# vislearn/HINT

Hardware: AMD Instinct MI355X
Metric: train_samples_per_sec (higher is better)
Workload: dtype f32; 1 GPU; power_hint_8: d=6, 8 recursive coupling blocks, c_internal=[140, 70, 35, 17], batch 4096 per GPU; global_batch=4096, parallelism=dp1, hip_graph=True, steps_per_graph=1, input=batch resident in the captured step's input buffer (no per-step copy), rccl_world_size=1, backend=none (one process), gradient_allreduce=none (one process: clamp + Adam ride in the weight gradients' final reduction)

## Files before the change

hint_amd/_lib.py:

```python
from __future__ import annotations

import ctypes as C
import os

_HERE = os.path.dirname(os.path.abspath(__file__))
LIB_PATH = os.environ.get("HINT_AMD_LIB") or os.path.join(_HERE, "lib", "libhint_amd.so")
ABI_VERSION = 8


class HintAmdError(RuntimeError):
    pass


class AdamSeg(C.Structure):
    _fields_ = [("p", C.c_void_p), ("g", C.c_void_p), ("m", C.c_void_p), ("v", C.c_void_p), ("n", C.c_int64)]


class NodeDesc(C.Structure):
    _fields_ = [("off", C.c_int32), ("D", C.c_int32), ("k", C.c_int32), ("r", C.c_int32),
                ("h", C.c_int32), ("depth", C.c_int32), ("p_off", C.c_int64 * 12)]


class MmdDesc(C.Structure):
    _fields_ = [("x", C.c_void_p), ("y", C.c_void_p), ("n_x", C.c_int32), ("n_y", C.c_int32), ("d", C.c_int32),
# ... 60 lines not shown
    "hint_build_info": (C.c_char_p, []),
    "hint_debug_set_prefetch": (C.c_int, [C.c_int]),
    "hint_debug_reload_knobs": (C.c_int, []),
    "hint_debug_last_lds_bytes": (C.c_int32, [C.c_int32]),
    "hint_plan_create": (C.c_int, [C.POINTER(NodeDesc), C.c_int32, C.c_int32, C.c_int32, C.c_float,
                                   C.POINTER(C.c_void_p)]),
    "hint_plan_check": (C.c_int, [C.POINTER(NodeDesc), C.c_int32, C.c_int32, C.c_int32, C.c_float,
                                  C.POINTER(C.c_int64)]),
    "hint_plan_destroy": (None, [C.c_void_p]),
    "hint_plan_param_floats": (C.c_int64, [C.c_void_p]),
    "hint_plan_packed_floats": (C.c_int64, [C.c_void_p]),
    "hint_plan_tape_floats": (C.c_int64, [C.c_void_p, C.c_int32]),
    "hint_plan_workspace_bytes": (C.c_size_t, [C.c_void_p, C.c_int32]),
    "hint_plan_lds_bytes": (C.c_int32, [C.c_void_p, C.c_int32]),
    "hint_plan_describe": (C.c_int, [C.c_void_p, C.c_int32, C.POINTER(C.c_int32)]),
    "hint_plan_dispatch": (C.c_int, [C.c_void_p, C.c_int32, C.POINTER(C.c_int32), C.c_int32]),
    "hint_plan_check_dispatch": (C.c_int, [C.POINTER(NodeDesc), C.c_int32, C.c_int32, C.c_int32, C.c_float, C.c_int32,
                                           C.c_int32, C.POINTER(C.c_int32), C.c_int32]),
    "hint_plan_paths": (C.c_int, [C.c_void_p, C.c_int32, C.POINTER(C.c_int32), C.c_int32]),
    "hint_plan_check_paths": (C.c_int, [C.POINTER(NodeDesc), C.c_int32, C.c_int32, C.c_int32, C.c_float, C.c_int32,
                                        C.c_int32, C.POINTER(C.c_int32), C.c_int32]),
    "hint_plan_check_digest": (C.c_int, [C.POINTER(NodeDesc), C.c_int32, C.c_int32, C.c_int32, C.c_float,
                                         C.POINTER(C.c_uint64), C.c_int32]),
    "hint_block_pack": (C.c_int, [C.c_void_p] * 4),
    "hint_pack_group_create": (C.c_int, [C.POINTER(C.c_void_p), C.POINTER(C.c_void_p), C.POINTER(C.c_void_p),
                                         C.c_int32, C.POINTER(C.c_void_p)]),
    "hint_pack_group_run": (C.c_int, [C.c_void_p, C.c_void_p]),
    "hint_pack_group_run_ex": (C.c_int, [C.c_void_p, C.c_void_p, C.c_int32, C.c_void_p, C.c_void_p, C.c_void_p]),
    "hint_pack_group_destroy": (None, [C.c_void_p]),
    "hint_block_forward": (C.c_int, [C.c_void_p] * 8 + [C.c_int32, C.c_void_p]),
    "hint_block_inverse": (C.c_int, [C.c_void_p] * 7 + [C.c_int32, C.c_void_p]),
    "hint_block_backward": (C.c_int, [C.c_void_p] * 11 + [C.c_int32, C.c_void_p, C.c_size_t, C.c_int32,
                                                          C.c_void_p]),
    "hint_block_forward_ex": (C.c_int, [C.c_void_p] * 11 + [C.c_int32, C.c_void_p]),
    "hint_block_inverse_ex": (C.c_int, [C.c_void_p] * 9 + [C.c_int32, C.c_void_p]),
    "hint_block_backward_ex": (C.c_int, [C.c_void_p] * 11 + [C.c_int32, C.c_void_p, C.c_size_t, C.c_void_p,
                                                             C.c_float, C.c_float, C.c_int32, C.c_void_p]),
    "hint_plan_inverse_workspace_bytes": (C.c_size_t, [C.c_void_p, C.c_int32]),
    "hint_block_inverse_backward": (C.c_int, [C.c_void_p] * 9 + [C.c_int32, C.c_void_p, C.c_size_t, C.c_void_p, C.c_int32,
                                                                 C.c_void_p]),
    "hint_chain_create": (C.c_int, [C.c_void_p, C.c_int32, C.c_int32, C.POINTER(C.c_void_p)]),
    "hint_chain_set_block": (C.c_int, [C.c_void_p, C.c_int32] + [C.c_void_p] * 5 + [C.c_size_t, C.c_void_p]),
    "hint_chain_commit": (C.c_int, [C.c_void_p]),
    "hint_chain_forward": (C.c_int, [C.c_void_p] * 8),
    "hint_chain_forward_noisy": (C.c_int, [C.c_void_p] * 7 + [C.c_float, C.c_void_p, C.c_void_p, C.c_void_p]),
    "hint_chain_backward": (C.c_int, [C.c_void_p] * 7 + [C.c_float, C.c_float, C.c_int32, C.c_void_p]),
# ... 77 lines not shown
```

hint_amd/csrc/hint_abi.cpp:

```cpp
#include "hint_host.hpp"

#include <atomic>

using namespace hint;

static thread_local std::string g_err;
static unsigned long long* g_stamp_buf = nullptr;

namespace hint {

static Knobs read_knobs() {
    Knobs k;
    auto get = [&](const char* name, int* out) {
        const char* e = std::getenv(name);
        if (!e || !*e) return false;
        *out = std::atoi(e);
        k.non_default += (k.non_default.empty() ? "" : " ") + std::string(name) + "=" + e;
        return true;
    };
    int v;
    if (get("HINT_PLAN_DUMP", &v)) k.plan_dump = v != 0;
    if (get("HINT_WL", &v)) k.wl = v != 0;
    if (get("HINT_WL_NR", &v)) k.wl_nr = v;
    if (get("HINT_SUB", &v)) k.sub = v != 0;
    if (get("HINT_NW", &v)) k.nw = v;
    if (get("HINT_LEAN", &v)) k.lean = v != 0;
    if (get("HINT_LEANW", &v)) k.leanw = v != 0;
    if (get("HINT_LEANW_MAX", &v)) k.leanw_max = std::min(std::max(v, 4), LEANW_MAX);
    if (get("HINT_FUSE_DW1", &v)) k.fuse_dw1 = v != 0;
    if (get("HINT_PF", &v)) k.pf = v != 0 ? 1 : 0;
    if (get("HINT_NO_BWD_FLY", &v)) k.no_bwd_fly = v != 0;
    if (get("HINT_DW_SPLITS", &v)) k.dw_splits = v;
    if (get("HINT_DW_SMALL", &v)) k.dw_small = v != 0 ? 1 : 0;
    if (get("HINT_ABLATION_OK", &v)) k.ablation_ok = v != 0;
    return k;
}
static std::mutex g_knobs_mu;
static Knobs* g_knobs = nullptr;
const Knobs& knobs() {
    std::lock_guard<std::mutex> lk(g_knobs_mu);
    if (!g_knobs) g_knobs = new Knobs(read_knobs());
    return *g_knobs;
}

int fail(const char* fmt, ...) {
    char buf[512];
    va_list ap;
    va_start(ap, fmt);
    vsnprintf(buf, sizeof buf, fmt, ap);
    va_end(ap);
    g_err = buf;
    return 1;
}
std::string& last_error_ref() { return g_err; }

const hint_plan* variant(const hint_plan* P, int B) {
// ... 175 lines not shown
    if (!knobs().ablation_ok) return fail("this is an ablation build (HINT_ABLATE_STORE): its gradients are wrong; set HINT_ABLATION_OK=1 for timing runs");
#endif

    const Dispatch D = dispatch(P, B, n_total);
    P = D.P;
    if ((parts & 1) && D.bwd == BWD_WL) {
        KArgs a = make_args(P, B, true);
        const int nr = D.nr;
        WlArgs w = P->wl_b[nr - 1];
        bool any_perm = one.perm != nullptr;
        if (chain_host) for (int i = 0; i < n_chain; ++i) any_perm = any_perm || chain_host[i].perm != nullptr;
        const int lds = lds_with_perms(P, plan_lds(P, true, nr), n_chain, any_perm, &a, true);
        w.off_perm = a.perm_lds;
        HIP_TRY(launch_wl_bwd(a, w, lds, D.grid, one, chain, n_chain, x, g_z, g_J, g_x, gz_scale, gJ_const, s));
    } else if (parts & 1) {
        KArgs a = make_args(P, B, true);
        const int lds = add_sink(P, P->lds_bwd, &a);
        g_last_lds[1].store(lds, std::memory_order_relaxed);
        HIP_TRY((D.bwd == BWD_FLY ? launch_bwd_fly : D.bwd == BWD_N3 ? launch_bwd_n3 : launch_bwd)(a, lds, D.grid, one, chain, n_chain, x, c,
                                                               g_z, g_J, g_x, g_c, gz_scale, gJ_const, s));
    }
    if (!(parts & 2)) return 0;
    const int splits = D.dw_splits, rows_per_wg = D.dw_rows;
    HIP_TRY(launch_wgrad(P->d_wjobs, P->n_wjobs, P->wsorted ? -P->n_wsmall - 1 : P->n_wsmall, splits, one, chain, n_chain, cb0, P->WT, P->ST, P->d, P->dc, P->n_levels, B,
                         rows_padded(B), rows_per_wg, act_stride(P, B), P->lean ? 0 : act_stride(P, B),
                         (P->lean ? 1 : 2) * act_stride(P, B) * 4 + bits_stride(P, B), P->param_floats, x, c, P->d_real,
                         accumulate, P->fuse_dw1 ? P->d_twmap : nullptr, P->tw_floats, ws_thin_off(P, B), D.grid,
                         P->num_cu, adam, D.dw_small, D.dw_wide, s));
    return 0;
}

}

static int apply(const hint_plan* P, bool rev, const float* params, const float* packed, const float* x,
                 const float* c, float* z, float* J, float* tape, const float* perm, const float* J_in,
                 float* loss_acc, int32_t B, void* stream, float noise = 0.f, const uint64_t* rng_state = nullptr,
                 float* x_noisy = nullptr) {
    const char* what = rev ? "inverse" : "forward";
    if (!P || !params || !packed || !x || !z || !J) return fail("hint_block_%s: null argument", what);
    if (P->dc > 0 && !c) return fail("hint_block_%s: plan has dc=%d but c is NULL", what, P->dc);
    if (B < 0) return fail("negative batch");
    if (B == 0) return 0;
    const Dispatch D = dispatch(P, B);
    P = D.P;
    ChainBlock one{};
    one.params = params; one.packed = packed; one.perm = perm;
    bind_tape(P, B, rev ? nullptr : tape, &one);
// ... 407 lines not shown
```

hint_amd/csrc/hint_dev.h:

```cpp
#pragma once
#include <stdint.h>

namespace hint {

constexpr int ROWS = 16;
constexpr int TILE = 16;
#ifndef HINT_MAX_NW
#define HINT_MAX_NW 8
#endif
#ifndef HINT_NTT
#define HINT_NTT 3
#endif
constexpr int MAX_NW = HINT_MAX_NW;
constexpr int NTT = HINT_NTT;
constexpr int MAX_RT = 4;
constexpr int MAX_CT = 12;
constexpr int LEANW_MAX = 28;
constexpr int LV_REGS = 4;

constexpr int PACK_SLACK = 1024;
struct PackSeg {
    int64_t dst;
    int64_t src;
    int32_t N, K;
// ... 47 lines not shown
struct Group {
    int32_t unit_begin, unit_end, ntiles, row_begin;
    int32_t ent_begin, ent_cnt, rng_begin, level;
    int32_t level_last, gcol0, gcols, lop_begin;
    int32_t level_first, tile_begin, wcol0, lean;
};
static_assert(sizeof(Group) == 64, "Group must be 4 x 16 bytes");

struct Ent {
    int16_t xcol, nquad;
    int16_t sl_ns, sl_nt;
    int32_t s_off, t_off;
};
static_assert(sizeof(Ent) == 16, "Ent must be 16 bytes");

struct LaneOp {
    int16_t sc_unit, sc_k;
    int16_t cp_ls, cp_lt;
    int16_t cp_gs, cp_gt;
    int32_t pad;
};
static_assert(sizeof(LaneOp) == 16, "LaneOp must be 16 bytes");

enum { WSRC_G1 = 0, WSRC_G2 = 1, WSRC_GST = 2, WSRC_A1 = 3, WSRC_A2 = 4, WSRC_X = 5, WSRC_C = 6, WSRC_A1R = 7, WSRC_G2R = 8 };
struct WJob {
    int32_t psrc, pcol, M, mw;
    int32_t qsrc, qcol, N, nw;
    int32_t qlevel, ldo;
    int32_t pmax, qmax;
    int64_t wofs;
    int64_t bofs;
    int32_t r_w1, r_b1;
    int32_t r_w3;
    int32_t r_cin, r_xoff;
    int32_t r_r, r_gcol;
    int32_t r_h, r_wcol;
    int32_t pad_[7];
};
static_assert(sizeof(WJob) == 128, "WJob must be 128 bytes");

struct RowRec {
    int32_t base1, base2;
    int32_t counts;
    int32_t aux;
    int32_t ocol;
    int32_t tile;
    int32_t slab;
// ... 95 lines not shown
```

hint_amd/csrc/hint_host.hpp:

```cpp
#pragma once
#include <hip/hip_runtime.h>

#include <algorithm>
#include <cmath>
#include <cstdarg>
#include <cstdio>
#include <cstdlib>
#include <cstring>
#include <mutex>
#include <string>
#include <vector>

#include "../../include/hint_amd.h"
#include "hint_dev.h"
#include "hint_adam.hpp"

namespace hint {
hipError_t launch_pack(const PackSeg* segs, const int2* ptiles, int n_tiles, const int32_t* bmap, int n_bias,
                       long bias_off, const float* params, float* packed, hipStream_t stream);
hipError_t launch_pack_many(const PackItem* items, int n_items, int grid, float* zero_buf, int zero_floats,
                            unsigned long long* rng_state, float* opt_state, hipStream_t stream);
hipError_t launch_zero(float* p, long n, int num_cu, hipStream_t stream);
hipError_t launch_inv_lane(int op, float* out, const float* g, const float* a, const float* b, const uint8_t* lower, long n, int d,
                           int num_cu, hipStream_t stream);
hipError_t launch_inv_minus(float* dst, const float* src, long n, int keep, int num_cu, hipStream_t stream);
hipError_t launch_inv_rowmat(const float* x, const float* P, float* y, long n, int d, int num_cu, hipStream_t stream);
hipError_t launch_apply(bool rev, bool fly, const KArgs& a, int lds_bytes, int grid, const ChainBlock& one,
                        const ChainBlock* chain, int n_chain, const float* x, const float* c, float* z, float* J,
                        const float* J_in, float* loss_acc, float noise, const unsigned long long* rng_state,
                        float* x_noisy, hipStream_t stream);
hipError_t launch_bwd(const KArgs& a, int lds_bytes, int grid, const ChainBlock& one, const ChainBlock* chain,
                      int n_chain, const float* x, const float* c, const float* g_z, const float* g_J,
                      float* g_x, float* g_c, float gz_scale, float gJ_const, hipStream_t stream);
hipError_t launch_wgrad(const WJob* jobs, int n_jobs, int n_small, int splits, const ChainBlock& one, const ChainBlock* chain,
                        int n_chain, int cb0, int WT, int ST, int d, int dc, int n_levels, int B, int Bp, int rows_per_wg,
                        int64_t act_stride, int64_t a2_off, int64_t bits_a2_off, int64_t param_floats, const float* x,
                        const float* c, const uint8_t* real, int accumulate, const int32_t* twmap, int tw_floats,
                        int64_t thin_slab_off, int thin_slabs, int num_cu, const AdamFuse* adam, bool small, bool wide,
                        hipStream_t stream);
hipError_t launch_bwd_n3(const KArgs& a, int lds_bytes, int grid, const ChainBlock& one, const ChainBlock* chain,
                         int n_chain, const float* x, const float* c, const float* g_z, const float* g_J,
                         float* g_x, float* g_c, float gz_scale, float gJ_const, hipStream_t stream);
hipError_t set_max_lds_apply(int bytes);
hipError_t launch_ext_coeff(const ExtArgs& a, hipStream_t stream);
hipError_t set_max_lds_bwd(int bytes);
hipError_t set_max_lds_bwd_n3(int bytes);
hipError_t launch_bwd_fly(const KArgs& a, int lds_bytes, int grid, const ChainBlock& one, const ChainBlock* chain,
                          int n_chain, const float* x, const float* c, const float* g_z, const float* g_J,
                          float* g_x, float* g_c, float gz_scale, float gJ_const, hipStream_t stream);
hipError_t set_max_lds_bwd_fly(int bytes);
hipError_t launch_wl_apply(bool rev, const KArgs& a, const WlArgs& w, int lds_bytes, int grid, const ChainBlock& one,
                           const ChainBlock* chain, int n_chain, const float* x, float* z, float* J, const float* J_in,
                           float* loss_acc, float noise, const unsigned long long* rng_state, float* x_noisy,
                           hipStream_t stream);
hipError_t launch_wl_bwd(const KArgs& a, const WlArgs& w, int lds_bytes, int grid, const ChainBlock& one,
                         const ChainBlock* chain, int n_chain, const float* x, const float* g_z, const float* g_J,
                         float* g_x, float gz_scale, float gJ_const, hipStream_t stream);
// ... 27 lines not shown

#ifdef HINT_STAMPS
static constexpr int LDS_LIMIT = 160 * 1024 - 32 * 1024 - 512;
#else
static constexpr int LDS_LIMIT = 160 * 1024;
#endif
static constexpr int LDS_ATTR = LDS_LIMIT;
static constexpr int PERM_LDS_MAX = 16 * 1024;
static constexpr int WS_SLACK = 64;

struct Knobs {
    bool plan_dump = false;
    bool wl = true;
    int wl_nr = 0;
    bool sub = true;
    int nw = 0;
    bool lean = true;
    bool leanw = true;
    bool fuse_dw1 = true;
    int pf = 1;
    bool no_bwd_fly = false;
    int dw_splits = 0;
    int dw_small = -1;
    int leanw_max = 12;
    bool ablation_ok = false;
    std::string non_default;
};
const Knobs& knobs();

}

using namespace hint;

struct hint_plan {
    int device = -1;
    int d = 0, dc = 0, n_nodes = 0, n_groups = 0, n_levels = 0, n_units = 0, n_wjobs = 0, n_wsmall = 0, wsorted = 0, n_ptiles = 0, nw = 8;
    float alpha = 0.f;
    int64_t param_floats = 0, packed_floats = 0;
    int WT = 0, ST = 0;
    int xld = 0, cld = 0, gld = 0, abuf_tiles = 0, slab_fwd = 0, slab_bwd = 0;
    int region_fwd = 0, region_bwd = 0;
    int stage_out = 1;
    int max_h = 0;
    int has_fly = 0;
    int lean = 0;
    int has_leanw = 0;
// ... 13 lines not shown
    int num_cu = 256;
    int meta_bytes = 0, units_off = 0, tmap_off = 0, ents_off = 0, rng_off = 0, lops_off = 0, n_bias = 0;
    void* d_meta = nullptr;
    int lop_cnt = 0;
    int max_slots = 0;
    LaneOp* d_lopsc = nullptr;
    RowRec* d_recs = nullptr;
    ThinRec* d_thins = nullptr;
    int total_tiles = 0;
    int total_rows = 0;
    int32_t* d_bmap = nullptr;
    uint8_t* d_real = nullptr;
    WJob* d_wjobs = nullptr;
    PackSeg* d_segs = nullptr;
    int2* d_ptiles = nullptr;
    hint_plan* alt4 = nullptr;
    std::vector<hint_node_desc> nodes;
    float clamp = 0.f;
    std::vector<int2> unit_w23;
    std::mutex inv_mu;
    std::vector<hint_plan*> inv_levels;
    uint8_t* d_inv_lower = nullptr;
    std::vector<uint64_t> digests;
    int tile_cap = 0, unit_waves = 0;
    int thin_spill_f = 0, thin_spill_b = 0;
    int max_r = 0, max_cin = 0;
    ~hint_plan();
};

namespace hint {

inline int plan_lds(const hint_plan* P, bool backward, int nr = 1) {
    if (P->wl) return 4 * (backward ? P->wl_b[nr - 1].off_perm : P->wl_f[nr - 1].off_perm);
    return backward ? P->lds_bwd : P->lds_fwd;
}
inline int rows_padded(int B) { return (B + ROWS - 1) / ROWS * ROWS; }

#ifdef HINT_STAMPS
void set_dw_stamps(unsigned long long* p);
#endif

bool l2_prefetch_on();
const hint_plan* variant(const hint_plan* P, int B);
int wl_nr_for(const hint_plan* Pv, int B);
int64_t tape_act_off(const hint_plan* P, int B);
int64_t act_stride(const hint_plan* P, int B);
// ... 28 lines not shown
```

hint_amd/csrc/hint_plan.cpp:

```cpp
#include "hint_host.hpp"

#include <memory>

using namespace hint;

#ifndef HINT_THIN_MFMA_MIN
#define HINT_THIN_MFMA_MIN 8
#endif
static constexpr int THIN_MFMA_MIN = HINT_THIN_MFMA_MIN;
static constexpr int THIN_LDS_MAX = 24 * 1024;
static constexpr int MAX_TAIL = 8;

struct Row { int unit, tb, ntt, slab3, slabv; long cost; };

static constexpr int GEN_NTT = 4;
static std::vector<Row> split_rows(const std::vector<Unit>& units, const Group& g, int nw, int ntt_max) {
    std::vector<int> nrows(g.unit_end - g.unit_begin);
    int total = 0;
    for (int ui = g.unit_begin; ui < g.unit_end; ++ui) { nrows[ui - g.unit_begin] = cdiv(units[ui].NT, ntt_max); total += nrows[ui - g.unit_begin]; }
    while (total < nw) {
        int best = -1; double bw = 0;
        for (int ui = g.unit_begin; ui < g.unit_end; ++ui) {
            const int nr = nrows[ui - g.unit_begin];
            if (nr >= units[ui].NT) continue;
// ... 845 lines not shown
    if (!bad) bad = check_records(b.groups, b.units, b.recs_f, b.recs_b, b.rng, nw);
    return bad ? fail("hint_plan_create: internal error (%s)", bad) : 0;
}

static void plan_wgrad_jobs(PlanBuild& b) {
    hint_plan* P = b.P.get();
    std::vector<WJob>& wjobs = b.wjobs;
    P->fuse_dw1 = P->tw_floats > 0 ? 1 : 0;
    make_wgrad_jobs(b);
    const bool small_on = knobs().dw_small >= 0 ? knobs().dw_small != 0 : P->n_sub > 0;
    const bool nat_on = !P->wl;
    auto is_small = [&](const WJob& j) { return j.mw <= 1 && j.nw <= 1 && (small_on || (nat_on && j.psrc == WSRC_G2R)); };
    std::stable_partition(wjobs.begin(), wjobs.end(), [&](const WJob& j) { return !is_small(j); });
    if (P->wl) {
        const auto nbig = std::count_if(wjobs.begin(), wjobs.end(), [&](const WJob& j) { return !is_small(j); });
        std::stable_sort(wjobs.begin(), wjobs.begin() + nbig, [](const WJob& x, const WJob& y) {
            return x.mw * std::max(1, x.nw) > y.mw * std::max(1, y.nw); });
        P->wsorted = 1;
    }
    P->n_wsmall = (int)std::count_if(wjobs.begin(), wjobs.end(), is_small);
    P->n_wjobs = (int)wjobs.size();
}

static void finish_tables(PlanBuild& b) {
    hint_plan* P = b.P.get();
    b.meta.assign(P->meta_bytes, 0);
    std::memcpy(b.meta.data(), b.groups.data(), b.groups.size() * sizeof(Group));
    std::memcpy(b.meta.data() + P->units_off, b.units.data(), b.units.size() * sizeof(Unit));
    if (!b.ents.empty()) std::memcpy(b.meta.data() + P->ents_off, b.ents.data(), b.ents.size() * sizeof(Ent));
    std::memcpy(b.meta.data() + P->rng_off, b.rng.data(), b.rng.size() * sizeof(int32_t));
    if (b.lops_lds) std::memcpy(b.meta.data() + P->lops_off, b.lc.data(), b.lc.size() * sizeof(LaneOp));
    P->total_rows = (int)b.recs_f.size();
    P->total_tiles = (int)b.thin_f.size();
    P->n_ptiles = (int)b.ptiles.size();
    b.thins = b.thin_f;
    b.thins.insert(b.thins.end(), b.thin_b.begin(), b.thin_b.end());
    b.thins.insert(b.thins.end(), b.thin_w.begin(), b.thin_w.end());
    b.recs = b.recs_f;
    b.recs.insert(b.recs.end(), b.recs_b.begin(), b.recs_b.end());
}

static uint64_t fnv1a(const void* p, size_t bytes) {
    uint64_t h = 0xcbf29ce484222325ull ^ (uint64_t)bytes;
    for (size_t i = 0; i < bytes; ++i) { h ^= static_cast<const unsigned char*>(p)[i]; h *= 0x100000001b3ull; }
    return h;
}
// ... 22 lines not shown
    for (const WlArgs* w : {&P->wl_f[0], &P->wl_f[1], &P->wl_b[0], &P->wl_b[1]})
        for (int i = 0; i < 13; ++i) v.push_back(reinterpret_cast<const int32_t*>(w)[i]);
    return digest(v);
}

static int upload_plan(PlanBuild& b) {
    hint_plan* P = b.P.get();
    hipDeviceProp_t prop;
    hipError_t e = hipGetDevice(&P->device);
    if (e == hipSuccess) e = hipGetDeviceProperties(&prop, P->device);
    if (e != hipSuccess) return fail("hint_plan_create: no device: %s", hipGetErrorString(e));
    P->num_cu = prop.multiProcessorCount > 0 ? prop.multiProcessorCount : 256;
    auto upload = [&e](void** dst, const auto& v) {
        const size_t bytes = v.size() * sizeof(v[0]);
        if (e == hipSuccess) e = hipMalloc(dst, std::max<size_t>(bytes, 16));
        if (e == hipSuccess && bytes) e = hipMemcpy(*dst, v.data(), bytes, hipMemcpyHostToDevice);
    };
    upload((void**)&P->d_meta, b.meta);
    upload((void**)&P->d_lopsc, b.lc);
    upload((void**)&P->d_thins, b.thins);
    upload((void**)&P->d_recs, b.recs);
    upload((void**)&P->d_bmap, b.bmap);
    upload((void**)&P->d_real, b.real);
    upload((void**)&P->d_wjobs, b.wjobs);
    if (!b.twmap.empty()) upload((void**)&P->d_twmap, b.twmap);
    upload((void**)&P->d_segs, b.segs);
    upload((void**)&P->d_ptiles, b.ptiles);
    if (e == hipSuccess) e = set_max_lds_apply(LDS_ATTR);
    if (e == hipSuccess) e = set_max_lds_bwd(LDS_ATTR);
    if (e == hipSuccess) e = set_max_lds_bwd_n3(LDS_ATTR);
    if (e == hipSuccess) e = set_max_lds_bwd_fly(LDS_ATTR);
    if (e == hipSuccess) e = set_max_lds_wl_apply(LDS_ATTR);
    if (e == hipSuccess) e = set_max_lds_wl_bwd(LDS_ATTR);
    return e == hipSuccess ? 0 : fail("hint_plan_create: device setup failed: %s", hipGetErrorString(e));
}

static int build_plan(const hint_node_desc* nodes, int32_t n_nodes, int32_t d, int32_t dc, float clamp, int nw,
                      int tile_cap, int unit_waves, bool host_only, hint_plan** out, bool* retry_smaller) {
    *retry_smaller = false;
    PlanBuild b(nodes, n_nodes, d, dc, clamp, nw, tile_cap, unit_waves);
    plan_subtree_levels(b);
    if (int st = plan_groups(b)) return st;
    if (int st = plan_lane_ops_and_sizes(b)) return st;
    classify_groups(b);
    plan_lds_regions(b);
    plan_fused_dw1(b);
    if (int st = plan_slots(b)) return st;
    if (int st = plan_lds_sizes(b, retry_smaller)) return st;
    if (int st = check_plan(b)) return st;
    plan_wgrad_jobs(b);
    finish_tables(b);
    if (host_only) b.P->digests = table_digests(b);
    else if (int st = upload_plan(b)) return st;
    *out = b.P.release();
    return 0;
}

static int pick_nw(int d) {
    int nw = 8;
    if (knobs().nw == 4 || knobs().nw == 8 || knobs().nw == 16) nw = std::min(knobs().nw, MAX_NW);
    while (nw < MAX_NW && ROWS * d > LV_REGS * 64 * nw) nw *= 2;
    return nw;
}

static int plan_for(const hint_node_desc* nodes, int32_t n_nodes, int32_t d, int32_t dc, float clamp, int nw, bool host_only,
                    hint_plan** out) {
    for (int unit_waves = nw; unit_waves >= 1; unit_waves /= 2)
        for (int tile_cap = 64; tile_cap >= 8; tile_cap -= 16) {
            bool retry = false;
            const int st = build_plan(nodes, n_nodes, d, dc, clamp, nw, tile_cap, unit_waves, host_only, out, &retry);
            if (st != 2) return st;
            if (!retry) break;
        }
// ... 92 lines not shown
    if (int st = host_plan(nodes, n_nodes, d, dc, clamp, &P)) return st;
    uint64_t all[2 * N_DIGESTS] = {};
    const hint_plan* both[2] = {P.get(), P->alt4};
    for (int v = 0; v < 2; ++v) {
        if (!both[v]) continue;
        std::copy(both[v]->digests.begin(), both[v]->digests.end(), all + v * N_DIGESTS);
        all[v * N_DIGESTS + N_TABLE_DIGESTS] = digest_scalars(both[v]);
    }
    std::copy(all, all + std::min<int>(n_out, 2 * N_DIGESTS), out);
    return 0;
}

int hint_plan_check_paths(const hint_node_desc* nodes, int32_t n_nodes, int32_t d, int32_t dc, float clamp, int32_t B,
                          int32_t num_cu, int32_t* out, int32_t n_out) {
    if (!out || B < 1 || num_cu < 1 || n_out < 1) return fail("hint_plan_check_paths: bad arguments");
    std::unique_ptr<hint_plan> P;
    if (int st = host_plan(nodes, n_nodes, d, dc, clamp, &P)) return st;
    P->num_cu = num_cu;
    if (P->alt4) P->alt4->num_cu = num_cu;
    paths_out(P.get(), B, out, n_out);
    return 0;
}

void hint_plan_destroy(hint_plan* P) { delete P; }

}
```

hint_amd/csrc/hint_wgrad.hip:

```cpp
#include "hint_device.hpp"
#include "hint_adam.hpp"

using namespace hint;

#ifndef HINT_DW_WAVES
#define HINT_DW_WAVES 2
#endif
constexpr int DW_WAVES = HINT_DW_WAVES;

#ifndef HINT_DW_BOUND
#define HINT_DW_BOUND , 4
#endif

#ifdef HINT_STAMPS
constexpr int DW_STAMP_IDS = 8;
static unsigned long long* h_dw_stamps = nullptr;
namespace hint { void set_dw_stamps(unsigned long long* p) { h_dw_stamps = p; } }
#define DW_STAMP(ID) { if (dw_stamps != nullptr) dw_st[ID] = __builtin_amdgcn_s_memtime(); }
#define DW_STAMP_WAIT(ID) { if (dw_stamps != nullptr) { asm volatile("s_waitcnt vmcnt(0) lgkmcnt(0)" ::: "memory"); dw_st[ID] = __builtin_amdgcn_s_memtime(); } }
#define DW_STAMP_FLUSH() { if (dw_stamps != nullptr && (threadIdx.x & 63) == 0) { \
    unsigned long long* o_ = dw_stamps + ((size_t)blockIdx.x * DW_WAVES + (threadIdx.x >> 6)) * DW_STAMP_IDS; \
    for (int i_ = 0; i_ < DW_STAMP_IDS; ++i_) o_[i_] = dw_st[i_]; } }
#else
#define DW_STAMP(ID) {}
// ... 329 lines not shown
                const int row_ = bb + 16 * t + 4 * i + kq;
                sa[t][i] = gs.ps.p[(size_t)min(row_, gs.ps.rows - 1) * gs.ps.ld + pc];
                sq[t][i] = ntn > 0 ? gs.qs.p[(size_t)min(row_, gs.qs.rows - 1) * gs.qs.ld + qc] : 0.f;
            }
#pragma unroll
        for (int i = 0; i < 4; ++i)
#pragma unroll
            for (int t = 0; t < NS; ++t) {
                ps8[t] += sa[t][i];
                acc[t / 3][t % 3] = mfma4(sa[t][i], sq[t][i], acc[t / 3][t % 3]);
            }
        bb += 16 * NS;
    }
#pragma unroll
    for (int t = 1; t < NS; ++t) {
        acc[0][0] += acc[t / 3][t % 3];
        acc[t / 3][t % 3] = zero4();
        ps8[0] += ps8[t];
    }
    psum[0] += ps8[0];
    cx.bb0 = bb;
}


template <bool SMALL, bool WIDE>
__global__ __launch_bounds__(DW_WAVES * 64 HINT_DW_BOUND) void hint_wgrad_kernel(
    const WJob* __restrict__ jobs, int n_jobs, int n_small, int splits, ChainBlock one, const ChainBlock* __restrict__ chain,
    int grid_pb, int cb0, int WT, int ST, int d, int dc, int n_levels, int B, int Bp, int rows_per_wg, int64_t act_stride,
    int64_t a2_off, int64_t bits_a2_off, int64_t param_floats, const float* __restrict__ x, const float* __restrict__ c
#ifdef HINT_STAMPS
    , unsigned long long* dw_stamps
#endif
    ) {
#ifdef HINT_STAMPS
    unsigned long long dw_st[DW_STAMP_IDS] = {0, 0, 0, 0, 0, 0, 0, 0};
#endif
    DW_STAMP(0)
    __shared__ float red[DW_WAVES][9][64][4];
    __shared__ float bred[DW_WAVES][3][16];

    const int n_big = n_jobs - n_small, items = n_big + (n_small + DW_WAVES - 1) / DW_WAVES;
    int cbi, bid;
    if (grid_pb > 0) {
        cbi = (int)blockIdx.x / grid_pb;
        bid = (int)blockIdx.x - cbi * grid_pb;
    } else {
        const int n_chain = (int)gridDim.x / -grid_pb;
        const int q = (int)blockIdx.x >> 3;
        cbi = q % n_chain;
        bid = (q / n_chain) * 8 + ((int)blockIdx.x & 7);
    }
    if (bid >= items * splits) return;
    const GBlock blk = chain_block(chain, one, cbi);
    const GLOBAL_AS float* xg = (const GLOBAL_AS float*)x;
    const GLOBAL_AS float* cg = (const GLOBAL_AS float*)c;
    const bool top = blk.perm != nullptr || (blk.x_in == nullptr && cbi + cb0 > 0);

    int item, split;
    if ((splits & 7) == 0) {
        const int xcd = bid & 7, t = bid >> 3;
        split = xcd + 8 * (t / items);
        item = t % items;
    } else {
        split = bid / items;
        item = bid % items;
    }
    const int tid = threadIdx.x, lane = tid & 63;
    const int wave = rfl(tid >> 6);
    const bool solo = SMALL && item >= n_big;
    const int jidx = solo ? n_big + (item - n_big) * DW_WAVES + wave : item;
    if (jidx >= n_jobs) return;
    const WJob job = jobs[jidx];
    DW_STAMP_WAIT(1)
    const int nl = lane & 15, kq = lane >> 4;
    const int ntm = job.mw, ntn = job.nw;
    const int b_begin = split * rows_per_wg;
    const int b_end = min(Bp, b_begin + rows_per_wg);

    f32x4 acc[3][3];
#pragma unroll
    for (int i = 0; i < 3; ++i)
#pragma unroll
        for (int j = 0; j < 3; ++j) acc[i][j] = zero4();
    float psum[3] = {0.f, 0.f, 0.f};
    const bool natural = job.psrc == WSRC_G2R;
    DwCtx cx;
    cx.nl = nl; cx.kq = kq;
    cx.step = solo ? 16 : 16 * DW_WAVES;
    cx.bb0 = b_begin + (solo ? 0 : wave * 16);
    cx.b_end = b_end;

// ... 210 lines not shown
                    if (r4[j] == 1) { ((float*)pp)[j] = p4[j]; ((float*)pm)[j] = m4[j]; ((float*)pv)[j] = v4[j]; }
            }
            continue;
        }
        f32x4 o = accumulate ? ((const f32x4*)g)[i4] : zero4();
        if (rl.x == 1) o.x += s.x;
        if (rl.y == 1) o.y += s.y;
        if (rl.z == 1) o.z += s.z;
        if (rl.w == 1) o.w += s.w;
        if (rl.x != 2 && rl.y != 2 && rl.z != 2 && rl.w != 2) {
            ((f32x4*)g)[i4] = o;
        } else {
            float* gp = g + 4 * i4;
            if (rl.x != 2) gp[0] = o.x;
            if (rl.y != 2) gp[1] = o.y;
            if (rl.z != 2) gp[2] = o.z;
            if (rl.w != 2) gp[3] = o.w;
        }
    }
}

namespace hint {

hipError_t launch_wgrad(const WJob* jobs, int n_jobs, int n_small, int splits, const ChainBlock& one, const ChainBlock* chain,
                        int n_chain, int cb0, int WT, int ST, int d, int dc, int n_levels, int B, int Bp, int rows_per_wg,
                        int64_t act_stride, int64_t a2_off, int64_t bits_a2_off, int64_t param_floats, const float* x,
                        const float* c, const uint8_t* real, int accumulate, const int32_t* twmap, int tw_floats,
                        int64_t thin_slab_off, int thin_slabs, int num_cu, const AdamFuse* adam, bool small, bool wide,
                        hipStream_t stream) {
    const bool interleave = n_small < 0;
    if (interleave) n_small = -n_small - 1;
#ifdef HINT_DW_SOLO_ALL
    n_small = n_jobs;
    small = n_jobs > 0;
#endif
    const int used = (n_jobs - n_small + (n_small + DW_WAVES - 1) / DW_WAVES) * splits;
    const int grid_pb = n_chain > 1 ? (used + 7) / 8 * 8 : used;
    if (used > 0) {
        const int gpb = (interleave && n_chain > 1 && (splits & 7) == 0) ? -grid_pb : grid_pb;
#ifdef HINT_STAMPS
#define HINT_DW_LAUNCH(S_, W_) hipLaunchKernelGGL((hint_wgrad_kernel<S_, W_>), dim3(grid_pb * n_chain), dim3(DW_WAVES * 64), 0, stream, jobs, n_jobs, n_small, splits, \
                               one, chain, gpb, cb0, WT, ST, d, dc, n_levels, B, Bp, rows_per_wg, act_stride, a2_off, bits_a2_off, param_floats, x, c, h_dw_stamps)
#else
#define HINT_DW_LAUNCH(S_, W_) hipLaunchKernelGGL((hint_wgrad_kernel<S_, W_>), dim3(grid_pb * n_chain), dim3(DW_WAVES * 64), 0, stream, jobs, n_jobs, n_small, splits, \
                               one, chain, gpb, cb0, WT, ST, d, dc, n_levels, B, Bp, rows_per_wg, act_stride, a2_off, bits_a2_off, param_floats, x, c)
#endif
        if (wide) { if (small) HINT_DW_LAUNCH(true, true); else HINT_DW_LAUNCH(false, true); }
        else if (small) HINT_DW_LAUNCH(true, false);
        else HINT_DW_LAUNCH(false, false);
#undef HINT_DW_LAUNCH
    }
    hipError_t e = hipGetLastError();
    if (e != hipSuccess) return e;
    int blocks_pb = (int)((param_floats / 4 + 255) / 256);
    const int cap = num_cu * 4 / (n_chain > 0 ? n_chain : 1);
    blocks_pb = blocks_pb < 1 ? 1 : (blocks_pb > cap && cap >= 1 ? cap : blocks_pb);
    const int thin_blocks = twmap != nullptr ? (tw_floats + 31) / 32 : 0;
    hipLaunchKernelGGL(hint_wreduce_kernel, dim3((blocks_pb + thin_blocks) * n_chain), dim3(256), 0, stream, one, chain, real,
                       param_floats, splits, accumulate, blocks_pb, twmap, tw_floats, thin_slab_off, thin_slabs, thin_blocks,
                       adam ? *adam : AdamFuse{});
    return hipGetLastError();
}

}
```

include/hint_amd.h:

```cpp
#ifndef HINT_AMD_H
#define HINT_AMD_H

#include <stddef.h>
#include <stdint.h>

#ifdef __cplusplus
extern "C" {
#endif

#define HINT_AMD_ABI_VERSION 8

enum { HINT_W1 = 0, HINT_B1 = 1, HINT_W2 = 2, HINT_B2 = 3, HINT_W3 = 4, HINT_B3 = 5 };

typedef struct hint_node_desc {
    int32_t off, D, k, r;
    int32_t h;
    int32_t depth;
    int64_t p_off[12];
} hint_node_desc;

typedef struct hint_plan hint_plan;

int hint_plan_create(const hint_node_desc* nodes, int32_t n_nodes, int32_t d, int32_t dc,
                     float clamp, hint_plan** out);

int hint_plan_check(const hint_node_desc* nodes, int32_t n_nodes, int32_t d, int32_t dc, float clamp,
                    int64_t* stats);
void hint_plan_destroy(hint_plan* plan);

int64_t hint_plan_param_floats(const hint_plan* plan);
int64_t hint_plan_packed_floats(const hint_plan* plan);
int64_t hint_plan_tape_floats(const hint_plan* plan, int32_t B);
size_t hint_plan_workspace_bytes(const hint_plan* plan, int32_t B);
int32_t hint_plan_lds_bytes(const hint_plan* plan, int32_t backward);
int hint_plan_describe(const hint_plan* plan, int32_t B, int32_t* out);

#define HINT_DISPATCH_FIELDS 20
int hint_plan_dispatch(const hint_plan* plan, int32_t B, int32_t* out, int32_t n_out);
int hint_plan_check_dispatch(const hint_node_desc* nodes, int32_t n_nodes, int32_t d, int32_t dc, float clamp, int32_t B,
                             int32_t num_cu, int32_t* out, int32_t n_out);
#define HINT_PATH_FIELDS 12
int hint_plan_paths(const hint_plan* plan, int32_t B, int32_t* out, int32_t n_out);
int hint_plan_check_paths(const hint_node_desc* nodes, int32_t n_nodes, int32_t d, int32_t dc, float clamp, int32_t B,
                          int32_t num_cu, int32_t* out, int32_t n_out);
#define HINT_PLAN_DIGESTS 12
int hint_plan_check_digest(const hint_node_desc* nodes, int32_t n_nodes, int32_t d, int32_t dc, float clamp, uint64_t* out,
                           int32_t n_out);

int hint_block_pack(const hint_plan* plan, const float* params, float* packed, void* stream);

typedef struct hint_pack_group hint_pack_group;
int hint_pack_group_create(const hint_plan* const* plans, const float* const* params,
                           float* const* packed, int32_t n, hint_pack_group** out);
int hint_pack_group_run(const hint_pack_group* group, void* stream);
int hint_pack_group_run_ex(const hint_pack_group* group, float* zero_buf, int32_t zero_floats,
                           uint64_t* rng_state, float* opt_state, void* stream);
void hint_pack_group_destroy(hint_pack_group* group);

int hint_block_forward(const hint_plan* plan, const float* params, const float* packed,
                       const float* x, const float* c, float* z, float* J, float* tape, int32_t B,
                       void* stream);
int hint_block_inverse(const hint_plan* plan, const float* params, const float* packed,
                       const float* z, const float* c, float* x, float* J, int32_t B, void* stream);
int hint_block_backward(const hint_plan* plan, const float* params, const float* packed,
                        const float* x, const float* tape, const float* c, const float* g_z,
                        const float* g_J, float* g_x, float* g_c, float* g_params,
                        int32_t accumulate, void* workspace, size_t workspace_bytes, int32_t B,
                        void* stream);

size_t hint_plan_inverse_workspace_bytes(const hint_plan* plan, int32_t B);
// ... 240 lines not shown
```

Measured before the change: 14.42 million samples/s.

## Add row-streaming MFMA path for small-rank W3 weight-gradient jobs

Weight-gradient jobs for the third coupling layer with r<=4 (GST x A2) are replaced by dedicated row jobs. Each wave streams batch rows and accumulates with 4x4x1 MFMA, covering up to 256 output columns and fusing the bias sum through shuffles. The goal is to avoid the general tiled wgrad path, which wastes work and LDS reductions on these very thin outer products. It is on by default when the plan has no sub-units, and adds a separate item class to the wgrad grid plus a host-side check API.

```diff
diff --git a/hint_amd/_lib.py b/hint_amd/_lib.py
--- a/hint_amd/_lib.py
+++ b/hint_amd/_lib.py
@@ -106,6 +106,8 @@
                                         C.c_int32, C.POINTER(C.c_int32), C.c_int32]),
     "hint_plan_check_digest": (C.c_int, [C.POINTER(NodeDesc), C.c_int32, C.c_int32, C.c_int32, C.c_float,
                                          C.POINTER(C.c_uint64), C.c_int32]),
+    "hint_plan_check_wjob": (C.c_int64, [C.POINTER(NodeDesc), C.c_int32, C.c_int32, C.c_int32, C.c_float, C.c_int32, C.c_int64,
+                                         C.c_int32]),
     "hint_block_pack": (C.c_int, [C.c_void_p] * 4),
     "hint_pack_group_create": (C.c_int, [C.POINTER(C.c_void_p), C.POINTER(C.c_void_p), C.POINTER(C.c_void_p),
                                          C.c_int32, C.POINTER(C.c_void_p)]),
diff --git a/hint_amd/csrc/hint_abi.cpp b/hint_amd/csrc/hint_abi.cpp
--- a/hint_amd/csrc/hint_abi.cpp
+++ b/hint_amd/csrc/hint_abi.cpp
@@ -32,6 +32,7 @@
     if (get("HINT_NO_BWD_FLY", &v)) k.no_bwd_fly = v != 0;
     if (get("HINT_DW_SPLITS", &v)) k.dw_splits = v;
     if (get("HINT_DW_SMALL", &v)) k.dw_small = v != 0 ? 1 : 0;
+    if (get("HINT_DW3_ROWS", &v)) k.dw3_rows = v != 0 ? 1 : 0;
     if (get("HINT_ABLATION_OK", &v)) k.ablation_ok = v != 0;
     return k;
 }
@@ -253,7 +254,7 @@
     }
     if (!(parts & 2)) return 0;
     const int splits = D.dw_splits, rows_per_wg = D.dw_rows;
-    HIP_TRY(launch_wgrad(P->d_wjobs, P->n_wjobs, P->wsorted ? -P->n_wsmall - 1 : P->n_wsmall, splits, one, chain, n_chain, cb0, P->WT, P->ST, P->d, P->dc, P->n_levels, B,
+    HIP_TRY(launch_wgrad(P->d_wjobs, P->n_ljobs, P->wsorted ? -P->n_lsmall - 1 : P->n_lsmall, P->n_rowj, splits, one, chain, n_chain, cb0, P->WT, P->ST, P->d, P->dc, P->n_levels, B,
                          rows_padded(B), rows_per_wg, act_stride(P, B), P->lean ? 0 : act_stride(P, B),
                          (P->lean ? 1 : 2) * act_stride(P, B) * 4 + bits_stride(P, B), P->param_floats, x, c, P->d_real,
                          accumulate, P->fuse_dw1 ? P->d_twmap : nullptr, P->tw_floats, ws_thin_off(P, B), D.grid,
diff --git a/hint_amd/csrc/hint_dev.h b/hint_amd/csrc/hint_dev.h
--- a/hint_amd/csrc/hint_dev.h
+++ b/hint_amd/csrc/hint_dev.h
@@ -93,7 +93,8 @@
 };
 static_assert(sizeof(LaneOp) == 16, "LaneOp must be 16 bytes");
 
-enum { WSRC_G1 = 0, WSRC_G2 = 1, WSRC_GST = 2, WSRC_A1 = 3, WSRC_A2 = 4, WSRC_X = 5, WSRC_C = 6, WSRC_A1R = 7, WSRC_G2R = 8 };
+enum { WSRC_G1 = 0, WSRC_G2 = 1, WSRC_GST = 2, WSRC_A1 = 3, WSRC_A2 = 4, WSRC_X = 5, WSRC_C = 6, WSRC_A1R = 7, WSRC_G2R = 8, WSRC_GSTR = 9 };
+constexpr int DW3R_COLS = 256;
 struct WJob {
     int32_t psrc, pcol, M, mw;
     int32_t qsrc, qcol, N, nw;
diff --git a/hint_amd/csrc/hint_host.hpp b/hint_amd/csrc/hint_host.hpp
--- a/hint_amd/csrc/hint_host.hpp
+++ b/hint_amd/csrc/hint_host.hpp
@@ -32,7 +32,7 @@
 hipError_t launch_bwd(const KArgs& a, int lds_bytes, int grid, const ChainBlock& one, const ChainBlock* chain,
                       int n_chain, const float* x, const float* c, const float* g_z, const float* g_J,
                       float* g_x, float* g_c, float gz_scale, float gJ_const, hipStream_t stream);
-hipError_t launch_wgrad(const WJob* jobs, int n_jobs, int n_small, int splits, const ChainBlock& one, const ChainBlock* chain,
+hipError_t launch_wgrad(const WJob* jobs, int n_jobs, int n_small, int n_rowj, int splits, const ChainBlock& one, const ChainBlock* chain,
                         int n_chain, int cb0, int WT, int ST, int d, int dc, int n_levels, int B, int Bp, int rows_per_wg,
                         int64_t act_stride, int64_t a2_off, int64_t bits_a2_off, int64_t param_floats, const float* x,
                         const float* c, const uint8_t* real, int accumulate, const int32_t* twmap, int tw_floats,
@@ -106,6 +106,7 @@
     bool no_bwd_fly = false;
     int dw_splits = 0;
     int dw_small = -1;
+    int dw3_rows = -1;
     int leanw_max = 12;
     bool ablation_ok = false;
     std::string non_default;
@@ -165,6 +166,8 @@
     std::vector<hint_plan*> inv_levels;
     uint8_t* d_inv_lower = nullptr;
     std::vector<uint64_t> digests;
+    std::vector<WJob> ljobs;
+    int n_ljobs = 0, n_lsmall = 0, n_rowj = 0;
     int tile_cap = 0, unit_waves = 0;
     int thin_spill_f = 0, thin_spill_b = 0;
     int max_r = 0, max_cin = 0;
diff --git a/hint_amd/csrc/hint_plan.cpp b/hint_amd/csrc/hint_plan.cpp
--- a/hint_amd/csrc/hint_plan.cpp
+++ b/hint_amd/csrc/hint_plan.cpp
@@ -891,6 +891,38 @@
     P->n_wjobs = (int)wjobs.size();
 }
 
+static void plan_launch_jobs(PlanBuild& b) {
+    hint_plan* P = b.P.get();
+    const bool rows_on = knobs().dw3_rows >= 0 ? knobs().dw3_rows != 0 : P->n_sub == 0;
+    auto covered = [&](const WJob& j) { return rows_on && j.psrc == WSRC_GST && j.qsrc == WSRC_A2 && j.r_r <= 4; };
+    P->ljobs.clear();
+    P->n_lsmall = 0;
+    for (size_t i = 0; i < b.wjobs.size(); ++i) {
+        if (covered(b.wjobs[i])) continue;
+        P->ljobs.push_back(b.wjobs[i]);
+        if ((int)i >= P->n_wjobs - P->n_wsmall) ++P->n_lsmall;
+    }
+    P->n_rowj = 0;
+    for (size_t ui = 0; rows_on && ui < b.units.size(); ++ui) {
+        const Unit& u = b.units[ui];
+        const hint_node_desc& n = b.nodes[b.unit_node[ui]];
+        if (n.r > 4) continue;
+        const int64_t* po = n.p_off + (int)(ui & 1) * 6;
+        for (int c0 = 0; c0 < n.h; c0 += DW3R_COLS) {
+            WJob j{};
+            j.psrc = WSRC_GSTR; j.pcol = u.gcol; j.M = n.r; j.mw = 1;
+            j.qsrc = WSRC_A2; j.qcol = u.wcol + c0; j.N = std::min(DW3R_COLS, n.h - c0); j.nw = cdiv(j.N, 64);
+            j.ldo = n.h; j.pmax = P->ST - 1; j.qmax = P->WT - 1;
+            j.wofs = po[HINT_W3] + c0;
+            j.bofs = c0 == 0 ? po[HINT_B3] : -1;
+            j.r_r = n.r; j.r_gcol = u.gcol; j.r_h = n.h; j.r_wcol = u.wcol;
+            P->ljobs.push_back(j);
+            ++P->n_rowj;
+        }
+    }
+    P->n_ljobs = (int)P->ljobs.size();
+}
+
 static void finish_tables(PlanBuild& b) {
     hint_plan* P = b.P.get();
     b.meta.assign(P->meta_bytes, 0);
@@ -959,7 +991,7 @@
     upload((void**)&P->d_recs, b.recs);
     upload((void**)&P->d_bmap, b.bmap);
     upload((void**)&P->d_real, b.real);
-    upload((void**)&P->d_wjobs, b.wjobs);
+    upload((void**)&P->d_wjobs, P->ljobs);
     if (!b.twmap.empty()) upload((void**)&P->d_twmap, b.twmap);
     upload((void**)&P->d_segs, b.segs);
     upload((void**)&P->d_ptiles, b.ptiles);
@@ -986,6 +1018,7 @@
     if (int st = plan_lds_sizes(b, retry_smaller)) return st;
     if (int st = check_plan(b)) return st;
     plan_wgrad_jobs(b);
+    plan_launch_jobs(b);
     finish_tables(b);
     if (host_only) b.P->digests = table_digests(b);
     else if (int st = upload_plan(b)) return st;
@@ -1124,6 +1157,25 @@
     return 0;
 }
 
+int64_t hint_plan_check_wjob(const hint_node_desc* nodes, int32_t n_nodes, int32_t d, int32_t dc, float clamp, int32_t variant,
+                             int64_t j, int32_t field) {
+    std::unique_ptr<hint_plan> P;
+    if (host_plan(nodes, n_nodes, d, dc, clamp, &P)) return INT64_MIN;
+    const hint_plan* V = variant ? P->alt4 : P.get();
+    if (!V) { fail("hint_plan_check_wjob: the plan has no 4-wavefront variant"); return INT64_MIN; }
+    if (j == -1 && field >= 0 && field < 5) {
+        const int64_t v[5] = {V->n_ljobs, V->n_lsmall, V->n_rowj, V->n_wjobs, V->n_wsmall};
+        return v[field];
+    }
+    if (j < 0 || j >= V->n_ljobs || field < 0 || field >= HINT_WJOB_FIELDS) {
+        fail("hint_plan_check_wjob: no job %lld / field %d (%d jobs)", (long long)j, field, V->n_ljobs);
+        return INT64_MIN;
+    }
+    const WJob& w = V->ljobs[(size_t)j];
+    const int64_t v[HINT_WJOB_FIELDS] = {w.psrc, w.pcol, w.M, w.mw, w.qsrc, w.qcol, w.N, w.nw, w.ldo, w.wofs, w.bofs, w.r_r, w.r_gcol, w.r_h, w.r_wcol};
+    return v[field];
+}
+
 void hint_plan_destroy(hint_plan* P) { delete P; }
 
 }
diff --git a/hint_amd/csrc/hint_wgrad.hip b/hint_amd/csrc/hint_wgrad.hip
--- a/hint_amd/csrc/hint_wgrad.hip
+++ b/hint_amd/csrc/hint_wgrad.hip
@@ -375,10 +375,79 @@
     cx.bb0 = bb;
 }
 
+template <int NQ, int AB>
+__device__ __forceinline__ void row_mma(f32x4 (&acc)[NQ], float a, const float (&b)[NQ]) {
+#pragma unroll
+    for (int q = 0; q < NQ; ++q) acc[q] = __builtin_amdgcn_mfma_f32_4x4x1f32(a, b[q], acc[q], 4, AB, 0);
+}
+constexpr int DW_ROWS_HALF = 8;
+template <int NQ>
+__device__ __forceinline__ void dw_rows(const WJob& job, const GBlock& blk, GLOBAL_AS float* slab, int b_begin, int b_end, int WT,
+                                        int ST, int64_t a2_off, int lane) {
+    constexpr int H = DW_ROWS_HALF;
+    f32x4 acc[NQ];
+#pragma unroll
+    for (int q = 0; q < NQ; ++q) acc[q] = zero4();
+    float asum = 0.f;
+    const int voff_a = (lane & 3) < job.M ? ((lane >> 2) * ST + job.pcol + (lane & 3)) * 4 : BUF_OOB;
+    int voff_b[NQ];
+#pragma unroll
+    for (int q = 0; q < NQ; ++q) voff_b[q] = 64 * q + lane < job.N ? (job.qcol + 64 * q + lane) * 4 : BUF_OOB;
+    const GLOBAL_AS float* gp = blk.wsGST;
+    const GLOBAL_AS float* ap = blk.actA1 + a2_off;
+    struct Half { float b[H][NQ]; };
+    auto load_a = [&](int bb) {
+        return buf_f32(__builtin_amdgcn_make_buffer_rsrc((void*)(gp + (size_t)bb * ST), 0, 16 * ST * 4, BUF_FLAGS), voff_a);
+    };
+    auto load_b = [&](int bb, int half) {
+        Half h;
+        const __amdgpu_buffer_rsrc_t r = __builtin_amdgcn_make_buffer_rsrc((void*)(ap + (size_t)bb * WT), 0, 16 * WT * 4, BUF_FLAGS);
+#pragma unroll
+        for (int k = 0; k < H; ++k)
+#pragma unroll
+            for (int q = 0; q < NQ; ++q) h.b[k][q] = as_f32(__builtin_amdgcn_raw_buffer_load_b32(r, voff_b[q], (H * half + k) * WT * 4, 0));
+        return h;
+    };
+#define DW_ROWS_MMA(A_, H_, AB0_) \
+    row_mma<NQ, AB0_ + 0>(acc, A_, H_.b[0]); row_mma<NQ, AB0_ + 1>(acc, A_, H_.b[1]); row_mma<NQ, AB0_ + 2>(acc, A_, H_.b[2]); \
+    row_mma<NQ, AB0_ + 3>(acc, A_, H_.b[3]); row_mma<NQ, AB0_ + 4>(acc, A_, H_.b[4]); row_mma<NQ, AB0_ + 5>(acc, A_, H_.b[5]); \
+    row_mma<NQ, AB0_ + 6>(acc, A_, H_.b[6]); row_mma<NQ, AB0_ + 7>(acc, A_, H_.b[7]);
+    static_assert(H == 8, "DW_ROWS_MMA names eight rows");
+    if (b_begin < b_end) {
+        const int last_bb = b_end - 16;
+        float a = load_a(b_begin);
+        Half h0 = load_b(b_begin, 0);
+        for (int bb = b_begin; bb < b_end; bb += 16) {
+            const Half h1 = load_b(bb, 1);
+            DW_ROWS_MMA(a, h0, 0)
+            const int nb = min(bb + 16, last_bb);
+            const float an = load_a(nb);
+            h0 = load_b(nb, 0);
+            DW_ROWS_MMA(a, h1, 8)
+            asum += a;
+            a = an;
+        }
+    }
+#undef DW_ROWS_MMA
+#pragma unroll
+    for (int q = 0; q < NQ; ++q) {
+        if (64 * q + lane >= job.N) continue;
+#pragma unroll
+        for (int i = 0; i < 4; ++i)
+            if (i < job.M) slab[job.wofs + (size_t)i * job.ldo + 64 * q + lane] = acc[q][i];
+    }
+    if (job.bofs >= 0) {
+        asum += __shfl_xor(asum, 4, 64);
+        asum += __shfl_xor(asum, 8, 64);
+        asum += __shfl_xor(asum, 16, 64);
+        asum += __shfl_xor(asum, 32, 64);
+        if (lane < job.M) slab[job.bofs + lane] = asum;
+    }
+}
 
 template <bool SMALL, bool WIDE>
 __global__ __launch_bounds__(DW_WAVES * 64 HINT_DW_BOUND) void hint_wgrad_kernel(
-    const WJob* __restrict__ jobs, int n_jobs, int n_small, int splits, ChainBlock one, const ChainBlock* __restrict__ chain,
+    const WJob* __restrict__ jobs, int n_jobs, int n_small, int n_rowj, int splits, ChainBlock one, const ChainBlock* __restrict__ chain,
     int grid_pb, int cb0, int WT, int ST, int d, int dc, int n_levels, int B, int Bp, int rows_per_wg, int64_t act_stride,
     int64_t a2_off, int64_t bits_a2_off, int64_t param_floats, const float* __restrict__ x, const float* __restrict__ c
 #ifdef HINT_STAMPS
@@ -392,7 +461,8 @@
     __shared__ float red[DW_WAVES][9][64][4];
     __shared__ float bred[DW_WAVES][3][16];
 
-    const int n_big = n_jobs - n_small, items = n_big + (n_small + DW_WAVES - 1) / DW_WAVES;
+    const int row_items = (n_rowj + DW_WAVES - 1) / DW_WAVES;
+    const int n_big = n_jobs - n_small - n_rowj, items = row_items + n_big + (n_small + DW_WAVES - 1) / DW_WAVES;
     int cbi, bid;
     if (grid_pb > 0) {
         cbi = (int)blockIdx.x / grid_pb;
@@ -420,6 +490,23 @@
     }
     const int tid = threadIdx.x, lane = tid & 63;
     const int wave = rfl(tid >> 6);
+    if (item < row_items) {
+        const int jr = n_jobs - n_rowj + item * DW_WAVES + wave;
+        if (jr >= n_jobs) return;
+        const WJob job = jobs[jr];
+        const int b_begin = split * rows_per_wg, b_end = min(Bp, b_begin + rows_per_wg);
+        GLOBAL_AS float* slab = blk.wsSlab + (size_t)split * param_floats;
+        switch (job.nw) {
+            case 1: dw_rows<1>(job, blk, slab, b_begin, b_end, WT, ST, a2_off, lane); break;
+            case 2: dw_rows<2>(job, blk, slab, b_begin, b_end, WT, ST, a2_off, lane); break;
+            case 3: dw_rows<3>(job, blk, slab, b_begin, b_end, WT, ST, a2_off, lane); break;
+            default: dw_rows<4>(job, blk, slab, b_begin, b_end, WT, ST, a2_off, lane); break;
+        }
+        DW_STAMP_WAIT(5)
+        DW_STAMP_FLUSH()
+        return;
+    }
+    item -= row_items;
     const bool solo = SMALL && item >= n_big;
     const int jidx = solo ? n_big + (item - n_big) * DW_WAVES + wave : item;
     if (jidx >= n_jobs) return;
@@ -676,7 +763,7 @@
 
 namespace hint {
 
-hipError_t launch_wgrad(const WJob* jobs, int n_jobs, int n_small, int splits, const ChainBlock& one, const ChainBlock* chain,
+hipError_t launch_wgrad(const WJob* jobs, int n_jobs, int n_small, int n_rowj, int splits, const ChainBlock& one, const ChainBlock* chain,
                         int n_chain, int cb0, int WT, int ST, int d, int dc, int n_levels, int B, int Bp, int rows_per_wg,
                         int64_t act_stride, int64_t a2_off, int64_t bits_a2_off, int64_t param_floats, const float* x,
                         const float* c, const uint8_t* real, int accumulate, const int32_t* twmap, int tw_floats,
@@ -685,18 +772,18 @@
     const bool interleave = n_small < 0;
     if (interleave) n_small = -n_small - 1;
 #ifdef HINT_DW_SOLO_ALL
-    n_small = n_jobs;
+    n_small = n_jobs - n_rowj;
     small = n_jobs > 0;
 #endif
-    const int used = (n_jobs - n_small + (n_small + DW_WAVES - 1) / DW_WAVES) * splits;
+    const int used = (n_jobs - n_small - n_rowj + (n_small + DW_WAVES - 1) / DW_WAVES + (n_rowj + DW_WAVES - 1) / DW_WAVES) * splits;
     const int grid_pb = n_chain > 1 ? (used + 7) / 8 * 8 : used;
     if (used > 0) {
         const int gpb = (interleave && n_chain > 1 && (splits & 7) == 0) ? -grid_pb : grid_pb;
 #ifdef HINT_STAMPS
-#define HINT_DW_LAUNCH(S_, W_) hipLaunchKernelGGL((hint_wgrad_kernel<S_, W_>), dim3(grid_pb * n_chain), dim3(DW_WAVES * 64), 0, stream, jobs, n_jobs, n_small, splits, \
+#define HINT_DW_LAUNCH(S_, W_) hipLaunchKernelGGL((hint_wgrad_kernel<S_, W_>), dim3(grid_pb * n_chain), dim3(DW_WAVES * 64), 0, stream, jobs, n_jobs, n_small, n_rowj, splits, \
                                one, chain, gpb, cb0, WT, ST, d, dc, n_levels, B, Bp, rows_per_wg, act_stride, a2_off, bits_a2_off, param_floats, x, c, h_dw_stamps)
 #else
-#define HINT_DW_LAUNCH(S_, W_) hipLaunchKernelGGL((hint_wgrad_kernel<S_, W_>), dim3(grid_pb * n_chain), dim3(DW_WAVES * 64), 0, stream, jobs, n_jobs, n_small, splits, \
+#define HINT_DW_LAUNCH(S_, W_) hipLaunchKernelGGL((hint_wgrad_kernel<S_, W_>), dim3(grid_pb * n_chain), dim3(DW_WAVES * 64), 0, stream, jobs, n_jobs, n_small, n_rowj, splits, \
                                one, chain, gpb, cb0, WT, ST, d, dc, n_levels, B, Bp, rows_per_wg, act_stride, a2_off, bits_a2_off, param_floats, x, c)
 #endif
         if (wide) { if (small) HINT_DW_LAUNCH(true, true); else HINT_DW_LAUNCH(false, true); }
diff --git a/include/hint_amd.h b/include/hint_amd.h
--- a/include/hint_amd.h
+++ b/include/hint_amd.h
@@ -46,6 +46,9 @@
 #define HINT_PLAN_DIGESTS 12
 int hint_plan_check_digest(const hint_node_desc* nodes, int32_t n_nodes, int32_t d, int32_t dc, float clamp, uint64_t* out,
                            int32_t n_out);
+#define HINT_WJOB_FIELDS 15
+int64_t hint_plan_check_wjob(const hint_node_desc* nodes, int32_t n_nodes, int32_t d, int32_t dc, float clamp, int32_t variant,
+                             int64_t j, int32_t field);
 
 int hint_block_pack(const hint_plan* plan, const float* params, float* packed, void* stream);
 
```

Measured after the change: 14.59 million samples/s (median of 6 runs). 1.01x the previous value.
